# markp-gc/ipu_ray_lib

Measured on AMD Instinct MI355X. Metric: rays/sec (ray casts/s: CompactBvh intersect+occluded calls, whole node), built-in scene 1440x1440 path-trace, higher is better.
Workload: dtype f32

## Files before the change

ipu_ray_lib_amd/csrc/ray_math.h:

```cpp
#pragma once

#include <stdint.h>
#include <string.h>
#include <math.h>

#if defined(__HIPCC__)
#define MI_HD __host__ __device__ __forceinline__
#else
#define MI_HD inline
#endif

namespace mi {

struct f3 { float x, y, z; };

MI_HD f3 mk(float x, float y, float z) { f3 r; r.x = x; r.y = y; r.z = z; return r; }
MI_HD f3 operator+(f3 a, f3 b) { return mk(a.x + b.x, a.y + b.y, a.z + b.z); }
MI_HD f3 operator-(f3 a, f3 b) { return mk(a.x - b.x, a.y - b.y, a.z - b.z); }
MI_HD f3 operator*(f3 a, f3 b) { return mk(a.x * b.x, a.y * b.y, a.z * b.z); }
MI_HD f3 operator*(f3 a, float s) { return mk(a.x * s, a.y * s, a.z * s); }
MI_HD f3 operator-(f3 a) { return mk(-a.x, -a.y, -a.z); }
MI_HD f3 abs3(f3 a) { return mk(fabsf(a.x), fabsf(a.y), fabsf(a.z)); }
MI_HD float dot(f3 a, f3 b) { return a.x * b.x + a.y * b.y + a.z * b.z; }
MI_HD float sqnorm(f3 a) { return a.x * a.x + a.y * a.y + a.z * a.z; }
// ... 117 lines not shown
MI_HD Box3 box_merge(Box3 a, const Box3& b) {
  a.lo.x = b.lo.x < a.lo.x ? b.lo.x : a.lo.x; a.lo.y = b.lo.y < a.lo.y ? b.lo.y : a.lo.y; a.lo.z = b.lo.z < a.lo.z ? b.lo.z : a.lo.z;
  a.hi.x = b.hi.x > a.hi.x ? b.hi.x : a.hi.x; a.hi.y = b.hi.y > a.hi.y ? b.hi.y : a.hi.y; a.hi.z = b.hi.z > a.hi.z ? b.hi.z : a.hi.z;
  return a;
}
MI_HD Box3 lbvh_scene_box(Box3 b) {
  b.lo = b.lo + mk(0.f, 0.f, 0.f); b.hi = b.hi + mk(0.f, 0.f, 0.f);
  return b;
}
MI_HD int lbvh_clz64(uint64_t x) {
#if defined(__HIP_DEVICE_COMPILE__)
  return __clzll((long long)x);
#else
  return x ? __builtin_clzll(x) : 64;
#endif
}
MI_HD int lbvh_delta(const uint64_t* keys, uint32_t n, uint32_t i, int64_t j) {
  if (j < 0 || j >= (int64_t)n) return -1;
  const uint64_t x = keys[i] ^ keys[j];
  return x ? lbvh_clz64(x) : 64 + lbvh_clz64((uint64_t)i ^ (uint64_t)j);
}
MI_HD void lbvh_node(const uint64_t* keys, uint32_t n, uint32_t i, uint32_t& first, uint32_t& last, uint32_t& split) {
  const int d = lbvh_delta(keys, n, i, (int64_t)i + 1) - lbvh_delta(keys, n, i, (int64_t)i - 1) >= 0 ? 1 : -1;
  const int dmin = lbvh_delta(keys, n, i, (int64_t)i - d);
  int64_t lmax = 2;
  while (lbvh_delta(keys, n, i, (int64_t)i + lmax * d) > dmin) lmax *= 2;
  int64_t l = 0;
  for (int64_t t = lmax / 2; t >= 1; t /= 2)
    if (lbvh_delta(keys, n, i, (int64_t)i + (l + t) * d) > dmin) l += t;
  const int64_t j = (int64_t)i + l * d;
  const int dnode = lbvh_delta(keys, n, i, j);
  int64_t s = 0;
  for (int64_t t = (l + 1) / 2;; t = (t + 1) / 2) {
    if (lbvh_delta(keys, n, i, (int64_t)i + (s + t) * d) > dnode) s += t;
    if (t == 1) break;
  }
  const int64_t g = (int64_t)i + s * d + (d < 0 ? -1 : 0);
  first = (uint32_t)(d > 0 ? (int64_t)i : j); last = (uint32_t)(d > 0 ? j : (int64_t)i); split = (uint32_t)g;
}
MI_HD double box_centre_dist2(const Box3& b) {
  const f3 c = (b.lo + b.hi) * .5f;
  return (double)c.x * c.x + (double)c.y * c.y + (double)c.z * c.z;
}

MI_HD double bvh_cost_term(uint16_t dx, uint16_t dy, uint16_t dz) {
  const double ex = (double)half_bits_to_float(dx), ey = (double)half_bits_to_float(dy), ez = (double)half_bits_to_float(dz);
  return (ex * ey + ey * ez) + ez * ex;
}
struct Cost2 { double all, leaf; };
MI_HD Cost2 cost_add(Cost2 a, Cost2 b) { Cost2 r; r.all = a.all + b.all; r.leaf = a.leaf + b.leaf; return r; }
constexpr uint32_t kCostBlock = 256;
template <class Sync>
MI_HD void cost_block_reduce(Cost2* v, uint32_t W, uint32_t lane, uint32_t lanes, Sync&& sync) {
  for (uint32_t s = W >> 1; s > 0; s >>= 1) {
    for (uint32_t i = lane; i < s; i += lanes) v[i] = cost_add(v[i], v[i + s]);
    sync();
  }
}
MI_HD uint32_t cost_blocks(uint32_t n, uint32_t W) { return n / W + (n % W ? 1u : 0u); }
constexpr double kCostBoxTest = 26.0, kCostPrimTest = 224.0;
MI_HD double bvh_cost_estimate(const double cost[3]) { return (kCostBoxTest * cost[0] + kCostPrimTest * cost[1]) / cost[2]; }

MI_HD void sincos_deg_table(float x, const float* tbl, float& s, float& c) {
  x = x * (float)(180.0 / 3.14159265358979323846264338327950288);
  const bool neg = x < 0.f;
  if (neg) x = -x;
  x = x - 360.f * floorf(x / 360.f);
  int ix = (int)(x + .5f);
  const float z = x - (float)ix;
  bool sneg = false, cneg = false;
  if (ix > 180) { sneg = true; cneg = true; ix -= 180; }
  if (ix > 90) { cneg = !cneg; ix = 180 - ix; }
  float sx = tbl[ix];
  if (sneg) sx = -sx;
  float cx = tbl[90 - ix];
  if (cneg) cx = -cx;
  const float sz = 1.74531263774940077459e-2f * z;
  const float cz = 1.f - 1.52307909153324666207e-4f * z * z;
  float y = sx * cz + cx * sz;
  if (neg) y = -y;
  s = y;
  c = cx * cz - sx * sz;
}

struct Rng { uint64_t s0, s1; };
MI_HD uint64_t rotl64(uint64_t x, int k) { return (x << k) | (x >> (64 - k)); }
MI_HD uint64_t splitmix64(uint64_t z) {
  z += 0x9e3779b97f4a7c15ull;
  z = (z ^ (z >> 30)) * 0xbf58476d1ce4e5b9ull;
  z = (z ^ (z >> 27)) * 0x94d049bb133111ebull;
  return z ^ (z >> 31);
}
MI_HD void rng_seed(Rng& r, uint64_t seed) { r.s0 = splitmix64(seed); r.s1 = splitmix64(r.s0); }
MI_HD uint64_t rng_next(Rng& r) {
  const uint64_t a = r.s0;
  uint64_t b = r.s1;
  const uint64_t out = rotl64(a * 5, 7) * 9;
  b ^= a;
  r.s0 = rotl64(a, 24) ^ b ^ (b << 16);
  r.s1 = rotl64(b, 37);
  return out;
}
MI_HD float rng_uniform01(Rng& r) {
  const uint64_t bits = (0x3FFull << 52) | (rng_next(r) >> 12);
  double d;
  __builtin_memcpy(&d, &bits, 8);
  return (float)(d - 1.0);
}

MI_HD uint32_t f2u_sat(float f) {
  if (!(f > 0.f)) return 0u;
  if (f >= 4294967296.f) return 0xFFFFFFFFu;
  return (uint32_t)f;
}
constexpr uint32_t kSegmentSamplesMin = 4, kSegmentSamplesMax = 64, kSegmentsPerPixel = 16;
MI_HD uint32_t segment_shift(uint32_t samplesPerPixel) {
  const uint32_t want = (samplesPerPixel + kSegmentsPerPixel - 1) / kSegmentsPerPixel;
  const uint32_t shift = want <= 1u ? 0u : 32u - (uint32_t)__builtin_clz(want - 1u);
  return shift < 2u ? 2u : shift > 6u ? 6u : shift;
}
MI_HD uint32_t segment_samples(uint32_t samplesPerPixel) { return 1u << segment_shift(samplesPerPixel); }
MI_HD void rng_seed_pixel_segment(Rng& r, uint64_t userSeed, float row, float col, uint32_t segment) {
  const uint64_t pix = ((uint64_t)f2u_sat(row) << 32) | (uint64_t)f2u_sat(col);
  rng_seed(r, (userSeed ^ ((pix + 1ull) * 0x9e3779b97f4a7c15ull)) ^ ((uint64_t)segment * 0xd1b54a32d192ed03ull));
}
MI_HD void rng_seed_pixel(Rng& r, uint64_t userSeed, float row, float col) { rng_seed_pixel_segment(r, userSeed, row, col, 0u); }

MI_HD float log_det(float x) {
  uint32_t b;
  __builtin_memcpy(&b, &x, 4);
  int e = (int)((b >> 23) & 0xFFu) - 126;
  const uint32_t mb = (b & 0x007FFFFFu) | 0x3F000000u;
  float m;
  __builtin_memcpy(&m, &mb, 4);
  if (m < 0.707106781186547524f) { e -= 1; m = m + m - 1.0f; }
  else { m = m - 1.0f; }
  float z = m * m;
  float y = 7.0376836292e-2f;
  y = y * m + -1.1514610310e-1f;
  y = y * m + 1.1676998740e-1f;
  y = y * m + -1.2420140846e-1f;
  y = y * m + 1.4249322787e-1f;
  y = y * m + -1.6668057665e-1f;
  y = y * m + 2.0000714765e-1f;
  y = y * m + -2.4999993993e-1f;
  y = y * m + 3.3333331174e-1f;
  y = y * m * z;
  const float fe = (float)e;
  y = y + -2.12194440e-4f * fe;
  y = y + -0.5f * z;
  z = m + y;
  z = z + 0.693359375f * fe;
  return z;
}
MI_HD void rng_gauss2(Rng& r, const float* sinTbl, float& g0, float& g1) {
  const float ua = rng_uniform01(r);
  const float ub = rng_uniform01(r);
  float w = 1.f - ua;
  if (w < 2.98023223876953125e-08f) w = 2.98023223876953125e-08f;
  const float rad = sqrtf(-2.f * log_det(w));
  float sn, cs;
  sincos_deg_table(6.283185307179586f * ub, sinTbl, sn, cs);
  g0 = rad * cs;
  g1 = rad * sn;
}

MI_HD f3 pixel_to_ray_dir(float x, float y, float w, float h, float tanTheta) {
  const float aspect = w / h;
  x = (x / w) - .5f;
  y = (y / h) - .5f;
  return normalized(mk(2.f * x * aspect * tanTheta, -2.f * y * tanTheta, -1.f));
}

MI_HD f3 offset_origin(f3 origin, f3 dir, f3 n) {
  const float m = (1.f + min_comp(abs3(origin))) * kRayEpsilon * copysignf(1.f, dot(n, dir));
  return origin + n * m;
}

MI_HD void sample_disc_concentric(float u1, float u2, const float* sinTbl, float& ox, float& oy) {
  const float ux = 2.f * u1 - 1.f, uy = 2.f * u2 - 1.f;
  if (ux == 0.f && uy == 0.f) { ox = ux; oy = uy; return; }
  const float piby4 = (float)(3.14159265358979323846264338327950288 / 4.0);
  const float piby2 = (float)(3.14159265358979323846264338327950288 / 2.0);
  const bool wide = fabsf(ux) > fabsf(uy);
  const float r = wide ? ux : uy;
  const float q = piby4 * ((wide ? uy : ux) / (wide ? ux : uy));
  const float th = wide ? q : piby2 - q;
  float s, c;
  sincos_deg_table(th, sinTbl, s, c);
  ox = r * c; oy = r * s;
}
MI_HD f3 cosine_sample_hemisphere(float u1, float u2, const float* sinTbl) {
  float x, y;
  sample_disc_concentric(u1, u2, sinTbl, x, y);
  const float z = sqrtf(fmaxf(0.f, 1.f - x * x - y * y));
  return mk(x, y, z);
}
MI_HD void diffuse_frame(f3 n, f3& xb, f3& yb) {
  const f3 a = abs3(n), sq = n * n;
  const bool wide = a.x > a.y;
  const float il = 1.f / sqrtf((wide ? sq.x : sq.y) + sq.z);
  const float m = (wide ? -n.z : n.z) * il;
  const float z = (wide ? n.x : -n.y) * il;
  xb = mk(wide ? m : 0.f, wide ? 0.f : m, z);
  yb = cross(n, xb);
}
MI_HD f3 diffuse_in_frame(f3 n, f3 xb, f3 yb, float u1, float u2, const float* sinTbl) {
  const f3 wi = cosine_sample_hemisphere(u1, u2, sinTbl);
  return mk(dot(mk(xb.x, yb.x, n.x), wi), dot(mk(xb.y, yb.y, n.y), wi), dot(mk(xb.z, yb.z, n.z), wi));
}
MI_HD f3 sample_diffuse(f3 n, float u1, float u2, const float* sinTbl) {
  f3 xb, yb;
  diffuse_frame(n, xb, yb);
  return diffuse_in_frame(n, xb, yb, u1, u2, sinTbl);
}
MI_HD f3 reflect_dir(f3 d, f3 n) {
  const float cosTheta = dot(d, n);
  return normalized(d - n * (cosTheta * 2.f));
}
MI_HD float schlick(float cosTheta, float ri) {
  float r0 = (1.f - ri) / (1.f + ri);
  r0 = r0 * r0;
  const float base = 1.f - cosTheta;
  const float base2 = base * base;
  const float base5 = base2 * base * base2;
  return r0 + (1.f - r0) * base5;
}
MI_HD f3 refract_dir(f3 dir, f3 n, float ndotr, float ri) {
  const float cosTheta = -ndotr;
  const f3 rPerp = (dir + n * cosTheta) * ri;
  const f3 rPar = n * -sqrtf(fabsf(1.f - sqnorm(rPerp)));
  return rPerp + rPar;
}
MI_HD bool dielectric(f3 dir, f3 n, float ri, float u1, f3& out) {
  if (dot(n, dir) > 0.f) n = -n; else ri = 1.f / ri;
  const float ndotr = dot(n, dir);
  const float cost1 = -ndotr;
  const float cost2 = 1.f - ri * ri * (1.f - cost1 * cost1);
  if (cost2 > 0.f && u1 > schlick(cost1, ri)) { out = refract_dir(dir, n, ndotr, ri); return true; }
  out = reflect_dir(dir, n);
  return false;
}
MI_HD bool roulette_stop(float u1, f3& tp) {
  const float p = min_comp(tp);
  if (p == 0.f || u1 > p) return true;
  tp = tp * (1.f / p);
  return false;
}

#define MI_SIN_TABLE_BITS \
  0x00000000u, 0x3c8ef859u, 0x3d0ef2c6u, 0x3d565e3au, 0x3d8edc7bu, 0x3db27eb6u, 0x3dd61305u, 0x3df996a2u, \
  0x3e0e8365u, 0x3e20305bu, 0x3e31d0d4u, 0x3e43636fu, 0x3e54e6cdu, 0x3e665992u, 0x3e77ba60u, 0x3e8483eeu, \
  0x3e8d2057u, 0x3e95b1beu, 0x3e9e377au, 0x3ea6b0dfu, 0x3eaf1d44u, 0x3eb77c01u, 0x3ebfcc6fu, 0x3ec80de9u, \
  0x3ed03fc9u, 0x3ed8616cu, 0x3ee0722fu, 0x3ee87171u, 0x3ef05e94u, 0x3ef838f7u, 0x3f000000u, 0x3f03d989u, \
  0x3f07a8cau, 0x3f0b6d77u, 0x3f0f2744u, 0x3f12d5e8u, 0x3f167918u, 0x3f1a108du, 0x3f1d9bfeu, 0x3f211b24u, \
  0x3f248dbbu, 0x3f27f37cu, 0x3f2b4c25u, 0x3f2e9772u, 0x3f31d522u, 0x3f3504f3u, 0x3f3826a7u, 0x3f3b39ffu, \
  0x3f3e3ebdu, 0x3f4134a6u, 0x3f441b7du, 0x3f46f30au, 0x3f49bb13u, 0x3f4c7360u, 0x3f4f1bbdu, 0x3f51b3f3u, \
  0x3f543bceu, 0x3f56b31du, 0x3f5919aeu, 0x3f5b6f51u, 0x3f5db3d7u, 0x3f5fe714u, 0x3f6208dau, 0x3f641901u, \
  0x3f66175eu, 0x3f6803cau, 0x3f69de1du, 0x3f6ba635u, 0x3f6d5becu, 0x3f6eff20u, 0x3f708fb2u, 0x3f720d81u, \
  0x3f737871u, 0x3f74d063u, 0x3f76153fu, 0x3f7746eau, 0x3f78654du, 0x3f797051u, 0x3f7a67e2u, 0x3f7b4bebu, \
  0x3f7c1c5cu, 0x3f7cd925u, 0x3f7d8235u, 0x3f7e1781u, 0x3f7e98fdu, 0x3f7f069eu, 0x3f7f605cu, 0x3f7fa62fu, \
  0x3f7fd814u, 0x3f7ff605u, 0x3f800000u, 0x3f7ff605u

}
```

ipu_ray_lib_amd/csrc/trace_wavefront.hpp:

```cpp
#pragma once

#include "trace_kernels.hpp"

namespace mi {

enum : uint32_t { PH_NODE = 0, PH_LEAF = 1, PH_SHADE = 2, PH_GEN = 3, PH_FETCH = 4, PH_DONE = 5 };
constexpr uint32_t kGenNode = 0x7FFFFFFDu, kFetchNode = 0x7FFFFFFEu, kDoneNode = 0x7FFFFFFFu;
static_assert(kGenNode > ((kLeafFlag >> 5) - 1u) << 5 && kDoneNode < kLeafFlag && kFetchNode == kGenNode + (PH_FETCH - PH_GEN) && kDoneNode == kGenNode + (PH_DONE - PH_GEN), "the parked phases lie between the largest byte offset and the leaf flag");

struct WaveTune { uint32_t leafAt, shadeAt, genAt, burst, keep8, dbl = 4, maxExtra = 6, leafThenNode = 1, prio = 1, leafP = 40, probe = 0;
  bool operator==(const WaveTune& o) const { return leafAt == o.leafAt && shadeAt == o.shadeAt && genAt == o.genAt && burst == o.burst && keep8 == o.keep8 && dbl == o.dbl && maxExtra == o.maxExtra && leafThenNode == o.leafThenNode && prio == o.prio && leafP == o.leafP && probe == o.probe; } };

struct WaveExtras {
  uint32_t sampleCount = 0;
  float* u = nullptr; float* v = nullptr;
  float* slotColor = nullptr; float* slotTp = nullptr;
  uint32_t* index = nullptr; uint32_t* count = nullptr;
  float azimuthRotation = 0.f;
  uint32_t fetchChunk = 0;
  float* segPart = nullptr;
  uint32_t segments = 1;
  uint32_t segBase = 0;
  const float2* coords = nullptr;
  uint32_t firstInSetup = 0;
};

__device__ __forceinline__ uint32_t lane_rank(unsigned long long mask) {
  return __builtin_amdgcn_mbcnt_hi((uint32_t)(mask >> 32), __builtin_amdgcn_mbcnt_lo((uint32_t)mask, 0u));
}

constexpr uint32_t kEnvChunk = 2048;
constexpr uint32_t kEnvBlock = 256;
constexpr uint32_t kEnvHole = 0xFFFFFFFFu;

constexpr WaveTune kDefaultTune = {8, 16, 24, 48, 3, 4, 6, 1, 1, 40, 0};
template <bool STATS, bool LDS_NODES, int BLOCK, int WAVES_PER_SIMD = 4, bool SPEC = false, int SLOTS = 2, bool FIXED_TUNE = false, bool DF = false, bool FAST = false, bool MERGE = true,
          bool BARY = true, bool ROT = false, bool HOT = false>
__global__ void __launch_bounds__(BLOCK, ((BLOCK == 256 || HOT) && WAVES_PER_SIMD > 4) ? WAVES_PER_SIMD : 1) path_trace_wavefront_kernel(DeviceScene sc, mi_trace_result* rays, uint32_t n,
                                                                   uint32_t* workCounter, uint32_t ldsNodeCount, WaveTune tuneArg, uint32_t tileStreamW, WaveExtras ex) {
  const WaveTune tune = FIXED_TUNE ? kDefaultTune : tuneArg;
  static_assert(!HOT || (MERGE && !SPEC && !FAST && !LDS_NODES && !DF), "HOT is a form of the default kernel's plain-render builds");
  const bool slots = (SLOTS == 2) ? (ex.slotColor != nullptr) : (SLOTS == 1);
  constexpr bool kFirstInSetup = SLOTS != 0 && MERGE && !SPEC && !FAST && !LDS_NODES && !DF && !HOT;
  __shared__ float sinTbl[92];
  constexpr uint32_t kMatCache = 16;
  struct __attribute__((aligned(16))) CachedMaterial { mi_material m; uint32_t pad[3]; };
  __shared__ CachedMaterial matS[kMatCache];
  const bool matsInLds = sc.numMaterials <= kMatCache;
  if (matsInLds) {
    for (uint32_t k = threadIdx.x; k < sc.numMaterials * 9u; k += blockDim.x)
      reinterpret_cast<uint32_t*>(&matS[k / 9u].m)[k % 9u] = reinterpret_cast<const uint32_t*>(sc.materials)[k];
  }
  extern __shared__ __attribute__((aligned(16))) unsigned char dynLds[];
  load_sin_table(sinTbl);
  if (LDS_NODES || HOT) {
    const uint4* src = reinterpret_cast<const uint4*>(sc.nodes);
    uint4* dst = reinterpret_cast<uint4*>(dynLds);
    for (uint32_t k = threadIdx.x; k < ldsNodeCount * 2; k += blockDim.x) dst[k] = src[k];
    __syncthreads();
  }
  const uint32_t hotBytes = HOT ? (ldsNodeCount << 5) : 0u;

  const uint32_t lane = threadIdx.x & 63;
  const uint32_t fetchChunk = ex.fetchChunk ? ex.fetchChunk : 64u;
  uint32_t chunkNext = 0, chunkEnd = 0;
  const uint32_t tiledCount = tileStreamW ? (n / (8u * tileStreamW)) * (8u * tileStreamW) : 0u;
  const uint32_t numNodes = sc.numNodes << 5;
  const uint32_t spp = ex.sampleCount ? ex.sampleCount : sc.samplesPerPixel;
  const bool segd = ex.segPart != nullptr || slots;
  const uint32_t segShift = (uint32_t)__builtin_amdgcn_readfirstlane((int)segment_shift(sc.samplesPerPixel)), segMask = (1u << segShift) - 1u;
  const uint32_t segs = segd ? ex.segments : 1u;
  const uint32_t items = n * segs;

  constexpr bool kPhInNode = !SPEC;
  uint32_t ph = PH_FETCH;
  uint32_t sample = 0, bounce = 0, node = kPhInNode ? kFetchNode : 0u, pendLeaf = 0;
  auto inNode = [&]() -> bool { return kPhInNode ? node < numNodes : ph == PH_NODE; };
  auto inLeaf = [&]() -> bool { return kPhInNode ? (int32_t)node < 0 : ph == PH_LEAF; };
  auto inShade = [&]() -> bool { return kPhInNode ? node - numNodes < kGenNode - numNodes : ph == PH_SHADE; };
  auto inGen = [&]() -> bool { return kPhInNode ? node == kGenNode : ph == PH_GEN; };
  auto inFetch = [&]() -> bool { return kPhInNode ? node == kFetchNode : ph == PH_FETCH; };
  auto park = [&](uint32_t p) { if (kPhInNode) node = kGenNode + (p - PH_GEN); else ph = p; };
  uint32_t pend1 = 0xFFFFFFFFu, pend1Node = 0, specNodes = 0;
  float prow = 0.f, pcol = 0.f;
  Rng rng; rng.s0 = rng.s1 = 0;
  f3 color = mk(0, 0, 0), tp = mk(1, 1, 1);
  f3 o = mk(0, 0, 0), d = mk(0, 0, -1), nrm = mk(0, 0, 1), inv = mk(0, 0, 0);
  f3 oi = mk(0, 0, 0);
  float slabPad = 0.f;
  Shear sh; sh.kz = 2; sh.sx = sh.sy = 0.f; sh.sz = 1.f;
  Hit hit; hit.t = kInf; hit.leaf = 0xFFFFFFFFu; hit.geomID = 0xFFFFu; hit.b0 = hit.b1 = hit.b2 = 0.f;
  uint32_t oFlags = 0;
  bool exactSlab = false;
  constexpr bool kCoordsFromStream = WAVES_PER_SIMD >= 7;
  constexpr uint32_t kColdWords = kCoordsFromStream ? 21u : 23u;
  __shared__ uint32_t coldLds[kColdWords * BLOCK];
  auto coldU = [&](uint32_t w) -> uint32_t& { return coldLds[((kCoordsFromStream && w > 2u) ? w - 2u : w) * BLOCK + threadIdx.x]; };
  auto coldF = [&](uint32_t w) -> float& { return reinterpret_cast<float*>(coldLds)[((kCoordsFromStream && w > 2u) ? w - 2u : w) * BLOCK + threadIdx.x]; };

  auto getPix = [&]() -> uint32_t { return coldU(0); };
  auto pathLoad = [&]() {
    rng.s0 = (uint64_t)coldU(8) | ((uint64_t)coldU(9) << 32); rng.s1 = (uint64_t)coldU(10) | ((uint64_t)coldU(11) << 32);
    color = mk(coldF(12), coldF(13), coldF(14)); tp = mk(coldF(15), coldF(16), coldF(17)); nrm = mk(coldF(18), coldF(19), coldF(20));
    { const uint32_t w = coldU(21); bounce = w >> 2; oFlags = w & 3u; } sample = coldU(22);
  };
  auto pathStore = [&]() {
    coldU(8) = (uint32_t)rng.s0; coldU(9) = (uint32_t)(rng.s0 >> 32); coldU(10) = (uint32_t)rng.s1; coldU(11) = (uint32_t)(rng.s1 >> 32);
    coldF(12) = color.x; coldF(13) = color.y; coldF(14) = color.z; coldF(15) = tp.x; coldF(16) = tp.y; coldF(17) = tp.z;
    coldF(18) = nrm.x; coldF(19) = nrm.y; coldF(20) = nrm.z;
    coldU(21) = (bounce << 2) | oFlags; coldU(22) = sample;
  };
  CastStats cs = {0, 0};
  uint32_t casts = 0, paths = 0;
  uint32_t itN = 0, itL = 0, itS = 0, itG = 0, lnN = 0, lnL = 0, lnS = 0, lnG = 0;
  uint32_t itH = 0, lnH = 0, itC = 0, lnC = 0;
  unsigned long long visHot = 0;
  uint32_t itQ = 0, lnQ = 0;
  unsigned long long tTrav = 0, tShade = 0, tGen = 0, tLoop0 = STATS ? __builtin_amdgcn_s_memtime() : 0ull;

  uint32_t envNext = 0, envEnd = 0, envFill = 0;
  auto pushEscaped = [&](bool envRay, uint32_t envSlot) {
    const unsigned long long mE = __ballot(envRay);
    if (!mE) return;
    const uint32_t firstE = (uint32_t)__ffsll((long long)mE) - 1u;
    const uint32_t nE = (uint32_t)__popcll(mE), room = envEnd - envNext;
    uint32_t fresh = 0;
    if (nE > room) {
      uint32_t b = 0;
      if (lane == firstE) b = atomicAdd(ex.count, kEnvChunk);
      fresh = (uint32_t)__builtin_amdgcn_readfirstlane((int)__shfl(b, firstE));
    }
    if (envRay) {
      const float twoPi = (float)(2.0 * 3.14159265358979323846264338327950288);
      const float invPi = (float)(1.0 / 3.14159265358979323846264338327950288);
// ... 213 lines not shown
                    if (node >= numNodes) pendLeaf = 0xFFFFFFFFu; else ph = PH_NODE;
                  } else ph = PH_SHADE;
                }
              }
            }
          } else
          if (inLeaf()) {
            if (STATS) cs.leaves++;
            const uint32_t at = node & ~kLeafFlag;
            if (!HOT) node = at;
            const uint32_t atLeaf = HOT ? (at >> 5) : (at >> 5) - 1u;
            const uint32_t recNode = HOT ? at : at - 32u;
            GLeaf L;
            if constexpr (ROT) {
              const GLeafBlock B = *reinterpret_cast<const GLeafBlock*>(reinterpret_cast<const char*>(sc.leavesRot) + ((recNode << 2) + sh.kz * 40u));
              L.type = B.type;
#pragma unroll
              for (int q = 0; q < 9; ++q) L.f[q] = B.f[q];
            } else {
              L = *reinterpret_cast<const GLeaf*>(reinterpret_cast<const char*>(sc.leaves) + (recNode << 1));
            }
            float t, b0 = 0.f, b1 = 0.f, b2 = 0.f;
            bool cand;
            const uint32_t kind = (HOT && ROT) ? (L.type & 31u) : leaf_kind(L);
            if constexpr (HOT) node = ROT ? (L.type & ~31u) : L.triBase;
            if (STATS) { const unsigned long long qm = __ballot(kind != LEAF_TRI); itQ += qm ? 1u : 0u; lnQ += (uint32_t)__popcll(qm); }
            if (kind == LEAF_TRI) {
              if constexpr (ROT) t = intersect_triangle<DF, true>(mk(L.f[0], L.f[1], L.f[2]), mk(L.f[3], L.f[4], L.f[5]), mk(L.f[6], L.f[7], L.f[8]), permute_kz(o, sh.kz), sh, b0, b1, b2);
              else
              t = FAST ? intersect_triangle_fast(mk(L.f[0], L.f[1], L.f[2]), mk(L.f[3], L.f[4], L.f[5]), mk(L.f[6], L.f[7], L.f[8]), o, sh, b0, b1, b2)
                       : intersect_triangle<DF>(mk(L.f[0], L.f[1], L.f[2]), mk(L.f[3], L.f[4], L.f[5]), mk(L.f[6], L.f[7], L.f[8]), o, sh, b0, b1, b2);
              cand = t > 0.f && t < kInf;
            } else if (kind == LEAF_SPHERE) {
              t = intersect_sphere(L, o, d, 0.f);
              cand = true;
            } else {
              t = intersect_disc(L, o, d);
              cand = true;
            }
            const bool closer = cand & (t > 0.f) & (t < hit.t);
            hit.t = closer ? t : hit.t; hit.leaf = closer ? atLeaf : hit.leaf;
            if constexpr (BARY) { hit.b0 = closer ? b0 : hit.b0; hit.b1 = closer ? b1 : hit.b1; hit.b2 = closer ? b2 : hit.b2; }
          }
          if (tune.leafThenNode) {
            if (STATS) { itN++; lnN += (uint32_t)__popcll(__ballot(inNode())); }
            if constexpr (SPEC) nodeStep();
            else if (inNode()) {
              if (anyExact) (void)nodeBodyT(std::true_type{}, std::false_type{});
              else (void)nodeBody();
            }
            ++steps;
          }
        }
        cN = (uint32_t)__popcll(__ballot(inNode()));
        cL = (uint32_t)__popcll(__ballot(inLeaf()));
        if (++steps >= tune.burst || (cN + cL) * 8u < startT * tune.keep8 || (cN + cL) == 0) break;
      }
      if (tune.prio == 1) __builtin_amdgcn_s_setprio(0); else if (tune.prio == 2) __builtin_amdgcn_s_setprio(1);
      if (STATS) tTrav += __builtin_amdgcn_s_memtime() - tq0;
    } else if (MERGE) {
      if (STATS) { itS++; lnS += cS + cG; }
      const unsigned long long tq1 = STATS ? __builtin_amdgcn_s_memtime() : 0ull;
      bool envRay = false, pathEnd = false, genNow = false, setup = false;
      uint32_t envSlot = 0;
      const bool wasShade = inShade(), wasGen = inGen();
      if (wasShade || wasGen) pathLoad();
      if (wasShade) {
        bool terminated = false;
        if (hit.leaf != 0xFFFFFFFFu) {
          const GLeaf L = sc.leaves[hit.leaf];
          constexpr bool kLeafFrame = !BARY && SLOTS == 0;
          f3 frX = mk(0.f, 0.f, 0.f), frY = frX;
          if constexpr (kLeafFrame) {
            if (sc.leafNormalsOrFrames != nullptr) {
              const GLeafFrame* fr = reinterpret_cast<const GLeafFrame*>(reinterpret_cast<const char*>(sc.leafNormalsOrFrames) + (hit.leaf << 5));
              frX = mk(fr->xb[0], fr->xb[1], fr->xb[2]); frY = mk(fr->yb[0], fr->yb[1], fr->yb[2]);
            }
          }
          hit.geomID = leaf_geom(L);
          coldU(6) = hit.leaf; coldF(7) = hit.t;
          o = o + d * hit.t;
          nrm = hit_normal(sc, hit, o);
          mi_material mat;
          if (matsInLds) { mat = matS[L.matIndex].m; asm volatile("" ::: "memory"); } else mat = sc.materials[L.matIndex];
          const f3 albedo = mk(mat.albedo.x, mat.albedo.y, mat.albedo.z);
          if (mat.emissive) color = color + tp * mk(mat.emission.x, mat.emission.y, mat.emission.z);
          if (mat.type == 0) {
            const float u1 = rng_uniform01(rng);
            const float u2 = rng_uniform01(rng);
            if constexpr (kLeafFrame) {
              f3 xb = frX, yb = frY;
              if ((frX.x == 0.f) & (frX.y == 0.f) & (frX.z == 0.f)) diffuse_frame(nrm, xb, yb);
              d = diffuse_in_frame(nrm, xb, yb, u1, u2, sinTbl);
            } else
            d = sample_diffuse(nrm, u1, u2, sinTbl);
            tp = tp * albedo;
          } else if (mat.type == 1) {
            d = reflect_dir(d, nrm);
            tp = tp * albedo;
          } else if (mat.type == 2) {
            const float u1 = rng_uniform01(rng);
            f3 nd2;
            const bool refracted = dielectric(d, nrm, mat.ior, u1, nd2);
            d = nd2;
            if (refracted) tp = tp * albedo;
          } else {
            const float qn = __builtin_nanf("");
            coldF(3) = coldF(3) * qn; coldF(4) = coldF(4) * qn; coldF(5) = coldF(5) * qn;
            oFlags |= MI_FLAG_ERROR;
          }
        } else {
          coldF(7) = kInf;
          oFlags |= MI_FLAG_ESCAPED;
          terminated = true;
        }
        if (!terminated && bounce > sc.rouletteStartDepth) {
          const float u1 = rng_uniform01(rng);
          if (roulette_stop(u1, tp)) terminated = true;
        }
        bounce++;
        if (bounce >= sc.maxPathLength) terminated = true;
        if (terminated) {
          const uint32_t pixNow = getPix();
          mi_trace_result* res = rays + pixNow;
          if (slots) {
            const size_t q = (size_t)sample * n + pixNow;
            ex.slotColor[3 * q] = color.x; ex.slotColor[3 * q + 1] = color.y; ex.slotColor[3 * q + 2] = color.z;
            envRay = (oFlags & MI_FLAG_ESCAPED) != 0;
            envSlot = (uint32_t)q;
            if (!envRay) ex.u[q] = -1.f;
          } else { coldF(3) = coldF(3) + color.x; coldF(4) = coldF(4) + color.y; coldF(5) = coldF(5) + color.z; }
          pathEnd = true;
          ++sample;
          const bool more = segd ? ((sample & segMask) != 0u && sample < spp) : (sample < spp);
          if (more) genNow = true;
          else if (segd && sample < spp) {
            if (!slots && ex.segPart) {
              float* part = ex.segPart + 3 * ((size_t)(((sample - 1u) >> segShift) - ex.segBase) * n + pixNow);
              part[0] = coldF(3); part[1] = coldF(4); part[2] = coldF(5);
            }
            park(PH_FETCH);
          } else {
            if (!slots && ex.segPart) {
              float* part = ex.segPart + 3 * ((size_t)(((sample - 1u) >> segShift) - ex.segBase) * n + pixNow);
              part[0] = coldF(3); part[1] = coldF(4); part[2] = coldF(5);
            } else
            if (!slots) res->rgb = {coldF(3), coldF(4), coldF(5)};
            uint32_t oPrim = MI_INVALID_PRIM, oGeom = MI_INVALID_GEOM;
            const uint32_t lastLeaf = coldU(6);
            if (lastLeaf != 0xFFFFFFFFu) { const GLeaf LL = sc.leaves[lastLeaf]; oPrim = LL.primID; oGeom = leaf_geom(LL); }
            mi_hit_record hr;
            hr.r.origin = {o.x, o.y, o.z}; hr.r.t_min = 0.f;
            hr.r.direction = {d.x, d.y, d.z}; hr.r.t_max = coldF(7);
            hr.prim_id = oPrim;
            hr.normal = {nrm.x, nrm.y, nrm.z};
            hr.throughput = {tp.x, tp.y, tp.z};
            hr.geom_id = (uint16_t)oGeom; hr.flags = (uint16_t)oFlags;
            res->h = hr;
            park(PH_FETCH);
          }
        } else {
          o = offset_origin(o, d, nrm);
          setup = true;
        }
      }
      if (slots) pushEscaped(envRay, envSlot);
      if (genNow || wasGen) {
        if constexpr (kCoordsFromStream) {
          const uint32_t e = coldU(0);
          if (ex.coords) { const float2 pc = ex.coords[e]; prow = pc.x; pcol = pc.y; } else { prow = rays[e].u; pcol = rays[e].v; }
        } else { prow = coldF(1); pcol = coldF(2); }
        float g0, g1;
        rng_gauss2(rng, sinTbl, g0, g1);
        const float jr = prow + sc.antiAliasScale * g0, jc = pcol + sc.antiAliasScale * g1;
        d = pixel_to_ray_dir(jc, jr, sc.imageWidth, sc.imageHeight, sc.tanTheta);
        o = mk(0.f, 0.f, 0.f);
        nrm = mk(0.f, 0.f, 1.f);
        coldU(6) = 0xFFFFFFFFu; coldF(7) = kInf;
        oFlags = 0;
        tp = mk(1.f, 1.f, 1.f);
        color = mk(0.f, 0.f, 0.f);
        bounce = 0;
        o = offset_origin(o, d, nrm);
        setup = true;
      }
      if (setup) {
        if (FAST) { inv = fast_inverse(d); sh = make_shear_fast(d, inv); }
        else {
          inv = mk(1.f / d.x, 1.f / d.y, 1.f / d.z);
          exactSlab = !(fabsf(inv.x) < kInf && fabsf(inv.y) < kInf && fabsf(inv.z) < kInf && fabsf(o.x) < kInf && fabsf(o.y) < kInf && fabsf(o.z) < kInf);
          sh = make_shear(d, inv);
        }
        if (FAST) fast_box_setup(o, inv, oi, slabPad);
        hit.t = kInf; hit.leaf = 0xFFFFFFFFu;
        { uint32_t seen; node = (root_start(sc, o, seen) << 5) + ((HOT && exactSlab) ? sc.exactBase : 0u); if (STATS) cs.nodes += seen; }
        if (!kPhInNode) ph = (numNodes > 0) ? PH_NODE : PH_SHADE;
        if constexpr (kFirstInSetup) {
          if (slots && ex.firstInSetup && inNode()) {
            const GNode nd = *reinterpret_cast<const GNode*>(reinterpret_cast<const char*>(sc.nodes) + node);
            if (STATS) cs.nodes++;
            const float ax = (nd.minx - o.x) * inv.x, bx = (nd.maxx - o.x) * inv.x;
            const float ay = (nd.miny - o.y) * inv.y, by = (nd.maxy - o.y) * inv.y;
            const float az = (nd.minz - o.z) * inv.z, bz = (nd.maxz - o.z) * inv.z;
            float t0 = fmaxf(fmaxf(fminf(ax, bx), fminf(ay, by)), fmaxf(fminf(az, bz), 0.f));
            float t1 = fminf(fminf(fminf(fmaxf(ax, bx), fmaxf(ay, by)), fmaxf(az, bz)) * kSlabScale, hit.t);
            if (exactSlab) {
              t0 = 0.f; t1 = hit.t;
              { float tmin = ax, tmax = bx; if (tmin > tmax) { const float w = tmin; tmin = tmax; tmax = w; } tmax *= kSlabScale; t0 = tmin > t0 ? tmin : t0; t1 = tmax < t1 ? tmax : t1; }
              { float tmin = ay, tmax = by; if (tmin > tmax) { const float w = tmin; tmin = tmax; tmax = w; } tmax *= kSlabScale; t0 = tmin > t0 ? tmin : t0; t1 = tmax < t1 ? tmax : t1; }
              { float tmin = az, tmax = bz; if (tmin > tmax) { const float w = tmin; tmin = tmax; tmax = w; } tmax *= kSlabScale; t0 = tmin > t0 ? tmin : t0; t1 = tmax < t1 ? tmax : t1; }
            }
            node = !(t0 > t1) ? nd.hit : nd.link;
          }
        }
      }
      if (wasShade || wasGen) pathStore();
      paths += (uint32_t)__popcll(__ballot(pathEnd));
      casts += (uint32_t)__popcll(__ballot(setup));
      if (STATS) tShade += __builtin_amdgcn_s_memtime() - tq1;
    } else if (run == 2) {
      if (STATS) { itS++; lnS += cS; }
      const unsigned long long tq1 = STATS ? __builtin_amdgcn_s_memtime() : 0ull;
      bool envRay = false;
      bool pathEnd = false;
      uint32_t envSlot = 0;
      if (inShade()) {
        pathLoad();
        bool terminated = false;
        if (hit.leaf != 0xFFFFFFFFu) {
          const GLeaf L = sc.leaves[hit.leaf];
          hit.geomID = leaf_geom(L);
          coldU(6) = hit.leaf; coldF(7) = hit.t;
          o = o + d * hit.t;
          nrm = hit_normal(sc, hit, o);
          mi_material mat;
          if (matsInLds) { mat = matS[L.matIndex].m; asm volatile("" ::: "memory"); } else mat = sc.materials[L.matIndex];
          const f3 albedo = mk(mat.albedo.x, mat.albedo.y, mat.albedo.z);
          if (mat.emissive) color = color + tp * mk(mat.emission.x, mat.emission.y, mat.emission.z);
          if (mat.type == 0) {
            const float u1 = rng_uniform01(rng);
            const float u2 = rng_uniform01(rng);
            d = sample_diffuse(nrm, u1, u2, sinTbl);
            tp = tp * albedo;
          } else if (mat.type == 1) {
            d = reflect_dir(d, nrm);
            tp = tp * albedo;
          } else if (mat.type == 2) {
            const float u1 = rng_uniform01(rng);
            f3 nd2;
            const bool refracted = dielectric(d, nrm, mat.ior, u1, nd2);
            d = nd2;
            if (refracted) tp = tp * albedo;
          } else {
            const float qn = __builtin_nanf("");
            coldF(3) = coldF(3) * qn; coldF(4) = coldF(4) * qn; coldF(5) = coldF(5) * qn;
            oFlags |= MI_FLAG_ERROR;
          }
        } else {
          coldF(7) = kInf;
          oFlags |= MI_FLAG_ESCAPED;
          terminated = true;
        }
        if (!terminated && bounce > sc.rouletteStartDepth) {
          const float u1 = rng_uniform01(rng);
          if (roulette_stop(u1, tp)) terminated = true;
        }
        bounce++;
        if (bounce >= sc.maxPathLength) terminated = true;
        if (terminated) {
          const uint32_t pixNow = getPix();
          mi_trace_result* res = rays + pixNow;
          if (slots) {
            const size_t q = (size_t)sample * n + pixNow;
            ex.slotColor[3 * q] = color.x; ex.slotColor[3 * q + 1] = color.y; ex.slotColor[3 * q + 2] = color.z;
            envRay = (oFlags & MI_FLAG_ESCAPED) != 0;
            envSlot = (uint32_t)q;
            if (!envRay) ex.u[q] = -1.f;
          } else { coldF(3) = coldF(3) + color.x; coldF(4) = coldF(4) + color.y; coldF(5) = coldF(5) + color.z; }
          pathEnd = true;
          ++sample;
          const bool more = segd ? ((sample & segMask) != 0u && sample < spp) : (sample < spp);
          if (more) park(PH_GEN);
          else if (segd && sample < spp) {
            if (!slots && ex.segPart) {
              float* part = ex.segPart + 3 * ((size_t)(((sample - 1u) >> segShift) - ex.segBase) * n + pixNow);
              part[0] = coldF(3); part[1] = coldF(4); part[2] = coldF(5);
            }
            park(PH_FETCH);
          } else {
            if (!slots && ex.segPart) {
              float* part = ex.segPart + 3 * ((size_t)(((sample - 1u) >> segShift) - ex.segBase) * n + pixNow);
              part[0] = coldF(3); part[1] = coldF(4); part[2] = coldF(5);
            } else
            if (!slots) res->rgb = {coldF(3), coldF(4), coldF(5)};
            uint32_t oPrim = MI_INVALID_PRIM, oGeom = MI_INVALID_GEOM;
            const uint32_t lastLeaf = coldU(6);
            if (lastLeaf != 0xFFFFFFFFu) { const GLeaf LL = sc.leaves[lastLeaf]; oPrim = LL.primID; oGeom = leaf_geom(LL); }
            mi_hit_record hr;
            hr.r.origin = {o.x, o.y, o.z}; hr.r.t_min = 0.f;
            hr.r.direction = {d.x, d.y, d.z}; hr.r.t_max = coldF(7);
            hr.prim_id = oPrim;
            hr.normal = {nrm.x, nrm.y, nrm.z};
            hr.throughput = {tp.x, tp.y, tp.z};
            hr.geom_id = (uint16_t)oGeom; hr.flags = (uint16_t)oFlags;
            res->h = hr;
            park(PH_FETCH);
          }
        } else {
          o = offset_origin(o, d, nrm);
          if (FAST) { inv = fast_inverse(d); sh = make_shear_fast(d, inv); }
          else {
            inv = mk(1.f / d.x, 1.f / d.y, 1.f / d.z);
            exactSlab = !(fabsf(inv.x) < kInf && fabsf(inv.y) < kInf && fabsf(inv.z) < kInf && fabsf(o.x) < kInf && fabsf(o.y) < kInf && fabsf(o.z) < kInf);
            sh = make_shear(d, inv);
          }
          if (FAST) fast_box_setup(o, inv, oi, slabPad);
          hit.t = kInf; hit.leaf = 0xFFFFFFFFu;
          { uint32_t seen; node = (root_start(sc, o, seen) << 5) + ((HOT && exactSlab) ? sc.exactBase : 0u); if (STATS) cs.nodes += seen; }
          if (!kPhInNode) ph = (numNodes > 0) ? PH_NODE : PH_SHADE;
        }
        pathStore();
      }
      { const uint32_t ended = (uint32_t)__popcll(__ballot(pathEnd)); paths += ended; casts += cS - ended; }
      if (slots) pushEscaped(envRay, envSlot);
      if (STATS) tShade += __builtin_amdgcn_s_memtime() - tq1;
    } else {
      if (STATS) { itG++; lnG += cG; }
      const unsigned long long tq2 = STATS ? __builtin_amdgcn_s_memtime() : 0ull;
      if (inGen()) {
        pathLoad();
        if constexpr (kCoordsFromStream) {
          const uint32_t e = coldU(0);
          if (ex.coords) { const float2 pc = ex.coords[e]; prow = pc.x; pcol = pc.y; } else { prow = rays[e].u; pcol = rays[e].v; }
        } else { prow = coldF(1); pcol = coldF(2); }
        float g0, g1;
// ... 70 lines not shown
```

Before: 21.57 billion.

## Precompute dielectric constants in LDS and specialise sincos/RNG shading math

Stores per-material dielectric constants (inverse IOR and both Schlick r0 values) next to each LDS-cached material and merges the mirror and glass shading branches into one helper that reads them, so the per-bounce divisions go away. Adds range-specialised sincos variants that skip the general modulo reduction for disc sampling and Gaussian angles, and swaps the xoshiro multiplies by 5 and 9 for v_lshl_add_u64 inline asm. A host-side exhaustive check confirms bitwise equality with the old math. The shade stage is small next to BVH traversal, so the effect on the metric may be small, and the larger LDS material entries could add some pressure.

After: 22.28 billion, median of 6. 1.03x the previous value.

```diff
diff --git a/ipu_ray_lib_amd/csrc/host/shade_consts_check.cpp b/ipu_ray_lib_amd/csrc/host/shade_consts_check.cpp
--- /dev/null
+++ b/ipu_ray_lib_amd/csrc/host/shade_consts_check.cpp
@@ -0,0 +1,201 @@
+#include "../ray_math.h"
+
+#include <atomic>
+#include <cmath>
+#include <cstdint>
+#include <cstdio>
+#include <cstring>
+#include <thread>
+#include <vector>
+
+namespace {
+
+using mi::f3;
+using mi::mk;
+
+uint32_t bits(float x) { uint32_t b; std::memcpy(&b, &x, 4); return b; }
+float from_bits(uint32_t b) { float x; std::memcpy(&x, &b, 4); return x; }
+
+uint64_t rngState = 0x9e3779b97f4a7c15ull;
+uint32_t rnd() { rngState ^= rngState << 13; rngState ^= rngState >> 7; rngState ^= rngState << 17; return (uint32_t)(rngState >> 16); }
+float rndUnit() { return (float)(rnd() >> 8) * (1.f / 16777216.f); }
+
+float sinTbl[92];
+std::atomic<long> failures{0};
+
+template <class F>
+void sweep(uint32_t lo, uint32_t hi, unsigned threads, F&& one) {
+  std::vector<std::thread> pool;
+  const uint64_t count = (uint64_t)hi - lo + 1u;
+  for (unsigned t = 0; t < threads; ++t) {
+    const uint32_t a = lo + (uint32_t)(count * t / threads), b = lo + (uint32_t)(count * (t + 1) / threads);
+    pool.emplace_back([a, b, &one]() { for (uint32_t v = a; v != b; ++v) one(from_bits(v)); });
+  }
+  for (auto& th : pool) th.join();
+}
+void check_small(float th) {
+  float ws, wc, gs, gc;
+  mi::sincos_deg_table(th, sinTbl, ws, wc);
+  mi::sincos_deg_table_small(th, sinTbl, gs, gc);
+  if ((bits(ws) != bits(gs) || bits(wc) != bits(gc)) && failures++ < 10)
+    std::printf("sincos_deg_table_small differs for th = %08x: want %08x %08x, got %08x %08x\n", bits(th), bits(ws), bits(wc), bits(gs), bits(gc));
+}
+void check_turn(float th) {
+  float ws, wc, gs, gc;
+  mi::sincos_deg_table(th, sinTbl, ws, wc);
+  mi::sincos_deg_table_turn(th, sinTbl, gs, gc);
+  if ((bits(ws) != bits(gs) || bits(wc) != bits(gc)) && failures++ < 10)
+    std::printf("sincos_deg_table_turn differs for th = %08x: want %08x %08x, got %08x %08x\n", bits(th), bits(ws), bits(wc), bits(gs), bits(gc));
+}
+
+void disc_general(float u1, float u2, float& ox, float& oy) {
+  const float ux = 2.f * u1 - 1.f, uy = 2.f * u2 - 1.f;
+  if (ux == 0.f && uy == 0.f) { ox = ux; oy = uy; return; }
+  const float piby4 = (float)(3.14159265358979323846264338327950288 / 4.0);
+  const float piby2 = (float)(3.14159265358979323846264338327950288 / 2.0);
+  const bool wide = fabsf(ux) > fabsf(uy);
+  const float r = wide ? ux : uy;
+  const float q = piby4 * ((wide ? uy : ux) / (wide ? ux : uy));
+  const float th = wide ? q : piby2 - q;
+  float s, c;
+  mi::sincos_deg_table(th, sinTbl, s, c);
+  ox = r * c; oy = r * s;
+}
+void gauss2_general(mi::Rng& r, float& g0, float& g1) {
+  const float ua = mi::rng_uniform01(r);
+  const float ub = mi::rng_uniform01(r);
+  float w = 1.f - ua;
+  if (w < 2.98023223876953125e-08f) w = 2.98023223876953125e-08f;
+  const float rad = sqrtf(-2.f * mi::log_det(w));
+  float sn, cs;
+  mi::sincos_deg_table(6.283185307179586f * ub, sinTbl, sn, cs);
+  g0 = rad * cs;
+  g1 = rad * sn;
+}
+void check_disc(float u1, float u2) {
+  float wx, wy, gx, gy;
+  disc_general(u1, u2, wx, wy);
+  mi::sample_disc_concentric(u1, u2, sinTbl, gx, gy);
+  if ((bits(wx) != bits(gx) || bits(wy) != bits(gy)) && failures++ < 10)
+    std::printf("sample_disc_concentric differs for u = %08x %08x: want %08x %08x, got %08x %08x\n", bits(u1), bits(u2), bits(wx), bits(wy), bits(gx), bits(gy));
+}
+void check_gauss(mi::Rng r) {
+  mi::Rng ra = r, rb = r;
+  float w0, w1, g0, g1;
+  gauss2_general(ra, w0, w1);
+  mi::rng_gauss2(rb, sinTbl, g0, g1);
+  if ((bits(w0) != bits(g0) || bits(w1) != bits(g1) || ra.s0 != rb.s0 || ra.s1 != rb.s1) && failures++ < 10)
+    std::printf("rng_gauss2 differs for state %016llx %016llx: want %08x %08x, got %08x %08x\n", (unsigned long long)r.s0, (unsigned long long)r.s1, bits(w0), bits(w1), bits(g0), bits(g1));
+}
+uint64_t draw_for(float u) {
+  if (u >= 1.f) return ~0ull << 12;
+  const double d = 1.0 + (double)u;
+  uint64_t b; std::memcpy(&b, &d, 8);
+  return (b & ((1ull << 52) - 1ull)) << 12;
+}
+uint64_t state_for(uint64_t out) {
+  const uint64_t x = out * 0x8E38E38E38E38E39ull;
+  return ((x >> 7) | (x << 57)) * 0xCCCCCCCCCCCCCCCDull;
+}
+mi::Rng rng_drawing(float ua, float ub) {
+  mi::Rng r;
+  r.s0 = state_for(draw_for(ua));
+  const uint64_t f = state_for(draw_for(ub)) ^ mi::rotl64(r.s0, 24);
+  const uint64_t b = f ^ (f << 16) ^ (f << 32) ^ (f << 48);
+  r.s1 = b ^ r.s0;
+  return r;
+}
+
+bool any_nan(f3 v) { return std::isnan(v.x) || std::isnan(v.y) || std::isnan(v.z); }
+bool same_dir(f3 w, f3 g, bool nanInput) {
+  const uint32_t a[3] = {bits(w.x), bits(w.y), bits(w.z)}, b[3] = {bits(g.x), bits(g.y), bits(g.z)};
+  for (int k = 0; k < 3; ++k) {
+    if (a[k] == b[k]) continue;
+    if (nanInput && std::isnan(from_bits(a[k])) && std::isnan(from_bits(b[k]))) continue;
+    return false;
+  }
+  return true;
+}
+void report(const char* what, f3 d, f3 n, float ior, float u1, f3 w, bool wf, f3 g, bool gf) {
+  if (failures++ < 10)
+    std::printf("%s differs for d = %08x %08x %08x, n = %08x %08x %08x, ior = %08x, u1 = %08x: want %08x %08x %08x (%d), got %08x %08x %08x (%d)\n", what, bits(d.x), bits(d.y), bits(d.z),
+                bits(n.x), bits(n.y), bits(n.z), bits(ior), bits(u1), bits(w.x), bits(w.y), bits(w.z), (int)wf, bits(g.x), bits(g.y), bits(g.z), (int)gf);
+}
+long bounces = 0;
+void check_bounce(f3 d, f3 n, float ior, float u1) {
+  const bool nanInput = any_nan(d) || any_nan(n) || std::isnan(ior) || std::isnan(u1);
+  const mi::DielectricConsts k = mi::dielectric_consts(ior);
+  f3 w, g;
+  const bool wf = mi::dielectric(d, n, ior, u1, w);
+  bool gf = mi::dielectric(d, n, ior, k, u1, g);
+  if (gf != wf || !same_dir(w, g, nanInput)) report("dielectric on constants", d, n, ior, u1, w, wf, g, gf);
+  gf = mi::dielectric_with(d, n, ior, mi::DielectricComputed{}, u1, g);
+  if (gf != wf || !same_dir(w, g, nanInput)) report("dielectric_with, computed ratio", d, n, ior, u1, w, wf, g, gf);
+  ++bounces;
+}
+
+}
+
+int main() {
+  { static const uint32_t tblBits[92] = {MI_SIN_TABLE_BITS}; std::memcpy(sinTbl, tblBits, sizeof sinTbl); }
+  unsigned threads = std::thread::hardware_concurrency();
+  threads = threads < 1u ? 1u : threads > 16u ? 16u : threads;
+
+  const uint32_t smallTop = bits(2.4f), turnTop = bits(6.2831855f);
+  sweep(0u, smallTop, threads, check_small);
+  sweep(0x80000000u, 0x80000000u | smallTop, threads, check_small);
+  sweep(0u, turnTop, threads, check_turn);
+  const unsigned long long angles = 2ull * ((unsigned long long)smallTop + 1u) + turnTop + 1u;
+
+  const float half = 0.5f, one = 1.f;
+  const std::vector<float> us = {0.f, half, one, from_bits(bits(half) - 1u), from_bits(bits(half) + 1u), from_bits(bits(half) - 2u), from_bits(bits(half) + 2u), 0.25f, 0.75f,
+                                 from_bits(bits(one) - 1u), from_bits(bits(one) - 2u), from_bits(0x33800000u), from_bits(0x34000000u), 0.125f, 0.875f, 0.1f, 0.9f, 1e-10f};
+  long discs = 0, gausses = 0;
+  for (float a : us) for (float b : us) { check_disc(a, b); ++discs; }
+  for (int k = 0; k < 2000000; ++k) {
+    const float a = rndUnit(), m = 1.f - a;
+    for (float b : {a, m, from_bits(bits(a) + 1u), from_bits(bits(m) + 1u), rndUnit(), half, 0.f, one}) { check_disc(a, b); check_disc(b, a); discs += 2; }
+  }
+  for (float a : us) for (float b : us) {
+    if (a == 1e-10f || b == 1e-10f) continue;
+    mi::Rng r = rng_drawing(a, b), probe = r;
+    const float da = mi::rng_uniform01(probe), db = mi::rng_uniform01(probe);
+    if ((bits(da) != bits(a) || bits(db) != bits(b)) && failures++ < 10) std::printf("the check's own state for draws %08x %08x draws %08x %08x\n", bits(a), bits(b), bits(da), bits(db));
+    check_gauss(r); ++gausses;
+  }
+  for (int k = 0; k < 4000000; ++k) {
+    mi::Rng r;
+    r.s0 = ((uint64_t)rnd() << 32) | rnd(); r.s1 = ((uint64_t)rnd() << 32) | rnd();
+    if (k & 1) r = rng_drawing(rndUnit(), (k & 2) ? from_bits(bits(one) - 1u - (rnd() & 7u)) : rndUnit());
+    check_gauss(r); ++gausses;
+  }
+
+  const float inf = INFINITY, qnan = from_bits(0x7FC00000u), nnan = from_bits(0xFFC00001u);
+  const float iors[] = {1.f, 1.52f, 0.5f, 1e-30f, 1e30f, 0.f, inf, qnan, 1.33f, 2.4f, -1.5f};
+  const float u1s[] = {0.f, 1.f, 0.5f, 0.04f, from_bits(bits(one) - 1u), from_bits(0x33800000u)};
+  const float comps[] = {0.f, -0.f, 1.f, -1.f, 0.70710678f, -0.70710678f, 0.6f, -0.8f, from_bits(1u), 1e-30f, -1e-20f, 1e19f, 3e38f, inf, -inf, qnan, nnan};
+  std::vector<f3> vs;
+  for (float x : comps) for (float y : comps) for (float z : comps) {
+    const int odd = (std::isfinite(x) && fabsf(x) <= 1.f ? 0 : 1) + (std::isfinite(y) && fabsf(y) <= 1.f ? 0 : 1) + (std::isfinite(z) && fabsf(z) <= 1.f ? 0 : 1);
+    if (odd <= 1) vs.push_back(mk(x, y, z));
+  }
+  for (size_t i = 0; i < vs.size(); ++i)
+    for (size_t j = i % 7; j < vs.size(); j += 7)
+      check_bounce(vs[i], vs[j], iors[(i + j) % 11], u1s[(i + 3 * j) % 6]);
+  for (int k = 0; k < 3000000; ++k) {
+    const f3 d = mi::normalized(mk(rndUnit() * 2.f - 1.f, rndUnit() * 2.f - 1.f, rndUnit() * 2.f - 1.f));
+    f3 n = mi::normalized(mk(rndUnit() * 2.f - 1.f, rndUnit() * 2.f - 1.f, rndUnit() * 2.f - 1.f));
+    if (k % 16 == 0) n = (k & 16) ? d : -d;
+    if (k % 16 == 1) n = mi::normalized(mi::cross(d, n));
+    const float ior = (k % 3 == 0) ? iors[k % 11] : (k % 3 == 1) ? 0.25f + 3.f * rndUnit() : from_bits(rnd());
+    const float u1 = (k % 5 == 0) ? u1s[k % 6] : rndUnit();
+    check_bounce(d, n, ior, u1);
+    check_bounce(d, -n, ior, u1);
+  }
+  for (int k = 0; k < 500000; ++k)
+    check_bounce(mk(from_bits(rnd()), from_bits(rnd()), from_bits(rnd())), mk(from_bits(rnd()), from_bits(rnd()), from_bits(rnd())), from_bits(rnd()), (k & 1) ? rndUnit() : from_bits(rnd()));
+
+  if (failures) { std::printf("shade_consts_check FAILED: %ld differences\n", failures.load()); return 1; }
+  std::printf("shade_consts_check OK: %llu angles, %ld disc samples, %ld gauss pairs, %ld bounces, all bits equal\n", angles, discs, gausses, bounces);
+  return 0;
+}
diff --git a/ipu_ray_lib_amd/csrc/ray_math.h b/ipu_ray_lib_amd/csrc/ray_math.h
--- a/ipu_ray_lib_amd/csrc/ray_math.h
+++ b/ipu_ray_lib_amd/csrc/ray_math.h
@@ -223,6 +223,33 @@
   s = y;
   c = cx * cz - sx * sz;
 }
+MI_HD void sincos_deg_reduced(float x, bool neg, const float* tbl, float& s, float& c) {
+  int ix = (int)(x + .5f);
+  const float z = x - (float)ix;
+  bool sneg = false, cneg = false;
+  if (ix > 180) { sneg = true; cneg = true; ix -= 180; }
+  if (ix > 90) { cneg = !cneg; ix = 180 - ix; }
+  float sx = tbl[ix];
+  if (sneg) sx = -sx;
+  float cx = tbl[90 - ix];
+  if (cneg) cx = -cx;
+  const float sz = 1.74531263774940077459e-2f * z;
+  const float cz = 1.f - 1.52307909153324666207e-4f * z * z;
+  float y = sx * cz + cx * sz;
+  if (neg) y = -y;
+  s = y;
+  c = cx * cz - sx * sz;
+}
+MI_HD void sincos_deg_table_small(float th, const float* tbl, float& s, float& c) {
+  float x = th * (float)(180.0 / 3.14159265358979323846264338327950288);
+  const bool neg = x < 0.f;
+  if (neg) x = -x;
+  sincos_deg_reduced(x, neg, tbl, s, c);
+}
+MI_HD void sincos_deg_table_turn(float th, const float* tbl, float& s, float& c) {
+  const float x = th * (float)(180.0 / 3.14159265358979323846264338327950288);
+  sincos_deg_reduced(x >= 360.f ? x - 360.f : x, false, tbl, s, c);
+}
 
 struct Rng { uint64_t s0, s1; };
 MI_HD uint64_t rotl64(uint64_t x, int k) { return (x << k) | (x >> (64 - k)); }
@@ -233,10 +260,17 @@
   return z ^ (z >> 31);
 }
 MI_HD void rng_seed(Rng& r, uint64_t seed) { r.s0 = splitmix64(seed); r.s1 = splitmix64(r.s0); }
+#if defined(__HIP_DEVICE_COMPILE__)
+MI_HD uint64_t mul5_u64(uint64_t a) { uint64_t r; asm("v_lshl_add_u64 %0, %1, 2, %1" : "=v"(r) : "v"(a)); return r; }
+MI_HD uint64_t mul9_u64(uint64_t a) { uint64_t r; asm("v_lshl_add_u64 %0, %1, 3, %1" : "=v"(r) : "v"(a)); return r; }
+#else
+MI_HD uint64_t mul5_u64(uint64_t a) { return a * 5; }
+MI_HD uint64_t mul9_u64(uint64_t a) { return a * 9; }
+#endif
 MI_HD uint64_t rng_next(Rng& r) {
   const uint64_t a = r.s0;
   uint64_t b = r.s1;
-  const uint64_t out = rotl64(a * 5, 7) * 9;
+  const uint64_t out = mul9_u64(rotl64(mul5_u64(a), 7));
   b ^= a;
   r.s0 = rotl64(a, 24) ^ b ^ (b << 16);
   r.s1 = rotl64(b, 37);
@@ -301,7 +335,7 @@
   if (w < 2.98023223876953125e-08f) w = 2.98023223876953125e-08f;
   const float rad = sqrtf(-2.f * log_det(w));
   float sn, cs;
-  sincos_deg_table(6.283185307179586f * ub, sinTbl, sn, cs);
+  sincos_deg_table_turn(6.283185307179586f * ub, sinTbl, sn, cs);
   g0 = rad * cs;
   g1 = rad * sn;
 }
@@ -328,7 +362,7 @@
   const float q = piby4 * ((wide ? uy : ux) / (wide ? ux : uy));
   const float th = wide ? q : piby2 - q;
   float s, c;
-  sincos_deg_table(th, sinTbl, s, c);
+  sincos_deg_table_small(th, sinTbl, s, c);
   ox = r * c; oy = r * s;
 }
 MI_HD f3 cosine_sample_hemisphere(float u1, float u2, const float* sinTbl) {
@@ -359,14 +393,17 @@
   const float cosTheta = dot(d, n);
   return normalized(d - n * (cosTheta * 2.f));
 }
-MI_HD float schlick(float cosTheta, float ri) {
-  float r0 = (1.f - ri) / (1.f + ri);
-  r0 = r0 * r0;
+MI_HD float schlick_r0(float ri) {
+  const float r0 = (1.f - ri) / (1.f + ri);
+  return r0 * r0;
+}
+MI_HD float schlick_from_r0(float cosTheta, float r0) {
   const float base = 1.f - cosTheta;
   const float base2 = base * base;
   const float base5 = base2 * base * base2;
   return r0 + (1.f - r0) * base5;
 }
+MI_HD float schlick(float cosTheta, float ri) { return schlick_from_r0(cosTheta, schlick_r0(ri)); }
 MI_HD f3 refract_dir(f3 dir, f3 n, float ndotr, float ri) {
   const float cosTheta = -ndotr;
   const f3 rPerp = (dir + n * cosTheta) * ri;
@@ -382,6 +419,38 @@
   out = reflect_dir(dir, n);
   return false;
 }
+struct DielectricConsts { float invIor, r0In, r0Out; };
+MI_HD DielectricConsts dielectric_consts(float ior) {
+  DielectricConsts k;
+  k.invIor = 1.f / ior;
+  k.r0In = schlick_r0(ior);
+  k.r0Out = schlick_r0(k.invIor);
+  return k;
+}
+struct DielectricComputed {};
+MI_HD void dielectric_ratio(float ior, const DielectricComputed&, bool inside, float& ri, float& r0) {
+  ri = inside ? ior : 1.f / ior;
+  r0 = schlick_r0(ri);
+}
+MI_HD void dielectric_ratio(float ior, const DielectricConsts& k, bool inside, float& ri, float& r0) {
+  ri = inside ? ior : k.invIor;
+  r0 = inside ? k.r0In : k.r0Out;
+}
+template <class K>
+MI_HD bool dielectric_with(f3 dir, f3 n, float ior, const K& k, float u1, f3& out) {
+  const bool inside = dot(n, dir) > 0.f;
+  if (inside) n = -n;
+  float ri, r0;
+  dielectric_ratio(ior, k, inside, ri, r0);
+  const float ndotr = dot(n, dir);
+  const float cost1 = -ndotr;
+  const float cost2 = 1.f - ri * ri * (1.f - cost1 * cost1);
+  const bool refracts = cost2 > 0.f && u1 > schlick_from_r0(cost1, r0);
+  if (refracts) out = refract_dir(dir, n, ndotr, ri);
+  else out = reflect_dir(dir, n);
+  return refracts;
+}
+MI_HD bool dielectric(f3 dir, f3 n, float ior, const DielectricConsts& k, float u1, f3& out) { return dielectric_with(dir, n, ior, k, u1, out); }
 MI_HD bool roulette_stop(float u1, f3& tp) {
   const float p = min_comp(tp);
   if (p == 0.f || u1 > p) return true;
diff --git a/ipu_ray_lib_amd/csrc/trace_wavefront.hpp b/ipu_ray_lib_amd/csrc/trace_wavefront.hpp
--- a/ipu_ray_lib_amd/csrc/trace_wavefront.hpp
+++ b/ipu_ray_lib_amd/csrc/trace_wavefront.hpp
@@ -33,6 +33,20 @@
 constexpr uint32_t kEnvBlock = 256;
 constexpr uint32_t kEnvHole = 0xFFFFFFFFu;
 
+template <class K>
+__device__ __forceinline__ void shade_specular(bool glass, float ior, const K& k, f3 albedo, Rng& rng, f3 nrm, f3& d, f3& tp) {
+  if (!glass) {
+    d = reflect_dir(d, nrm);
+    tp = tp * albedo;
+  } else {
+    const float u1 = rng_uniform01(rng);
+    f3 nd;
+    const bool refracted = dielectric_with(d, nrm, ior, k, u1, nd);
+    d = nd;
+    if (refracted) tp = tp * albedo;
+  }
+}
+
 constexpr WaveTune kDefaultTune = {8, 16, 24, 48, 3, 4, 6, 1, 1, 40, 0};
 template <bool STATS, bool LDS_NODES, int BLOCK, int WAVES_PER_SIMD = 4, bool SPEC = false, int SLOTS = 2, bool FIXED_TUNE = false, bool DF = false, bool FAST = false, bool MERGE = true,
           bool BARY = true, bool ROT = false, bool HOT = false>
@@ -44,12 +58,16 @@
   constexpr bool kFirstInSetup = SLOTS != 0 && MERGE && !SPEC && !FAST && !LDS_NODES && !DF && !HOT;
   __shared__ float sinTbl[92];
   constexpr uint32_t kMatCache = 16;
-  struct __attribute__((aligned(16))) CachedMaterial { mi_material m; uint32_t pad[3]; };
+  struct __attribute__((aligned(16))) CachedMaterial { mi_material m; DielectricConsts k; };
+  static_assert(sizeof(CachedMaterial) == 48 && sizeof(mi_material) == 36, "a staged material is three 16-byte reads");
   __shared__ CachedMaterial matS[kMatCache];
   const bool matsInLds = sc.numMaterials <= kMatCache;
   if (matsInLds) {
-    for (uint32_t k = threadIdx.x; k < sc.numMaterials * 9u; k += blockDim.x)
-      reinterpret_cast<uint32_t*>(&matS[k / 9u].m)[k % 9u] = reinterpret_cast<const uint32_t*>(sc.materials)[k];
+    for (uint32_t k = threadIdx.x; k < sc.numMaterials * 9u; k += blockDim.x) {
+      const uint32_t w = reinterpret_cast<const uint32_t*>(sc.materials)[k];
+      reinterpret_cast<uint32_t*>(&matS[k / 9u].m)[k % 9u] = w;
+      if (k % 9u == offsetof(mi_material, ior) / 4u) matS[k / 9u].k = dielectric_consts(__uint_as_float(w));
+    }
   }
   extern __shared__ __attribute__((aligned(16))) unsigned char dynLds[];
   load_sin_table(sinTbl);
@@ -429,7 +447,8 @@
           o = o + d * hit.t;
           nrm = hit_normal(sc, hit, o);
           mi_material mat;
-          if (matsInLds) { mat = matS[L.matIndex].m; asm volatile("" ::: "memory"); } else mat = sc.materials[L.matIndex];
+          DielectricConsts matK = {0.f, 0.f, 0.f};
+          if (matsInLds) { mat = matS[L.matIndex].m; matK = matS[L.matIndex].k; asm volatile("" ::: "memory"); } else mat = sc.materials[L.matIndex];
           const f3 albedo = mk(mat.albedo.x, mat.albedo.y, mat.albedo.z);
           if (mat.emissive) color = color + tp * mk(mat.emission.x, mat.emission.y, mat.emission.z);
           if (mat.type == 0) {
@@ -442,15 +461,9 @@
             } else
             d = sample_diffuse(nrm, u1, u2, sinTbl);
             tp = tp * albedo;
-          } else if (mat.type == 1) {
-            d = reflect_dir(d, nrm);
-            tp = tp * albedo;
-          } else if (mat.type == 2) {
-            const float u1 = rng_uniform01(rng);
-            f3 nd2;
-            const bool refracted = dielectric(d, nrm, mat.ior, u1, nd2);
-            d = nd2;
-            if (refracted) tp = tp * albedo;
+          } else if (mat.type == 1 || mat.type == 2) {
+            if (matsInLds) shade_specular(mat.type == 2, mat.ior, matK, albedo, rng, nrm, d, tp);
+            else shade_specular(mat.type == 2, mat.ior, DielectricComputed{}, albedo, rng, nrm, d, tp);
           } else {
             const float qn = __builtin_nanf("");
             coldF(3) = coldF(3) * qn; coldF(4) = coldF(4) * qn; coldF(5) = coldF(5) * qn;
@@ -581,7 +594,8 @@
           o = o + d * hit.t;
           nrm = hit_normal(sc, hit, o);
           mi_material mat;
-          if (matsInLds) { mat = matS[L.matIndex].m; asm volatile("" ::: "memory"); } else mat = sc.materials[L.matIndex];
+          DielectricConsts matK = {0.f, 0.f, 0.f};
+          if (matsInLds) { mat = matS[L.matIndex].m; matK = matS[L.matIndex].k; asm volatile("" ::: "memory"); } else mat = sc.materials[L.matIndex];
           const f3 albedo = mk(mat.albedo.x, mat.albedo.y, mat.albedo.z);
           if (mat.emissive) color = color + tp * mk(mat.emission.x, mat.emission.y, mat.emission.z);
           if (mat.type == 0) {
@@ -589,15 +603,9 @@
             const float u2 = rng_uniform01(rng);
             d = sample_diffuse(nrm, u1, u2, sinTbl);
             tp = tp * albedo;
-          } else if (mat.type == 1) {
-            d = reflect_dir(d, nrm);
-            tp = tp * albedo;
-          } else if (mat.type == 2) {
-            const float u1 = rng_uniform01(rng);
-            f3 nd2;
-            const bool refracted = dielectric(d, nrm, mat.ior, u1, nd2);
-            d = nd2;
-            if (refracted) tp = tp * albedo;
+          } else if (mat.type == 1 || mat.type == 2) {
+            if (matsInLds) shade_specular(mat.type == 2, mat.ior, matK, albedo, rng, nrm, d, tp);
+            else shade_specular(mat.type == 2, mat.ior, DielectricComputed{}, albedo, rng, nrm, d, tp);
           } else {
             const float qn = __builtin_nanf("");
             coldF(3) = coldF(3) * qn; coldF(4) = coldF(4) * qn; coldF(5) = coldF(5) * qn;
```
